# SegataLab/metamlst

Hardware: AMD Instinct MI355X
Metric: Mreads/s aligned+ST-typed, metamlstDB_2022; ST concordance vs CPU ref (higher is better)
Workload: dtype int32

## Files before the change

### metamlst_amd/csrc/mlst_engine.hip

```cpp
#include <hip/hip_runtime.h>
#include <algorithm>
#include <cmath>
#include <cstdarg>
#include <cstdio>
#include <cstdlib>
#include <cstring>
#include <cstddef>
#include <functional>
#include <atomic>
#include <memory>
#include <mutex>
#include <string>
#include <thread>
#include <vector>
#include <chrono>
#include <unistd.h>

#include "mlst.h"
#include "mlst_debug.h"
#include "bgzf_host.h"
#include "inflate_dev.h"
#include "inflate_wave.h"
#include "inflate_lane.h"
#include "inflate_canon.h"
// ... 91 lines not shown
    u64 sv_wgmax;
    u64 cnt[MLST_CNT_N];
    u64 rt_next;
    u64 rt_parked;
    u64 rt_ring_full;
    u64 pad_[13];
    u64 ext_q2[EXT_Q][16];
};
#define IS_SINGLE 1
#define IS_DONE   2
#define IS_ACC    4
struct KParams {
    int minscore, max_xm, min_read_len, minqual, match_bonus, n_penalty, open_p, ext_p, gbar, band_w, trig, quirk, clip;
};
#if defined(__HIP_DEVICE_COMPILE__)
#define GLOBAL_AS __attribute__((address_space(1)))
#else
#define GLOBAL_AS
#endif
template <typename T> struct GP {
    T* p;
#if defined(__HIP_DEVICE_COMPILE__)
    typedef __attribute__((address_space(1))) T G;
#else
    typedef T G;
#endif
    __host__ __device__ GP& operator=(T* q) { p = q; return *this; }
    template <typename I> __device__ G& operator[](I i) const { return ((G*)p)[i]; }
    __device__ G* operator->() const { return (G*)p; }
    __host__ __device__ operator T*() const { return p; }
    __device__ G* g() const { return (G*)p; }
};

struct EngineDev {
    GP<const u32> arena; GP<const u32> planes; GP<const u32> nmask; GP<const u16> allele_len; GP<const u32> allele_locus; GP<const LocusDev> loci;
    GP<const uint4> sieve; u32 sieve_mask;
    GP<const u32> bitmap;
    GP<const u32> gbitmap; u32 gbitmap_bits;
    GP<const u64> keys; GP<const u32> vals; GP<const u32> posts; u32 table_mask;
    GP<const int> floor_tab; GP<const u8> pen_tab;
    u32 n_alleles, n_loci;
    GP<const HapRec> hap_rec; GP<const u32> hap_blk; GP<const u32> hap_id;
    GP<u64> acc64;
    GP<long long> sum_score; GP<u32> n_hits; GP<u64> locus_len; GP<u64> locus_first;
    GP<Counters> ctr;
    GP<u32> ret_bases; GP<u8> ret_quals; GP<u16> ret_len; GP<u64> ret_ridx; GP<u32> ret_nrec;
    GP<u32> ret_cpos;
    GP<u32> ret_mate; GP<u32> ret_item0; GP<u8> ret_nitems;
    GP<ItemDev> items; GP<u8> item_state; GP<u32> res; GP<u64> dp_list;
    u64 cap_ret, cap_items, cap_res, cap_dp;
};

#define TIE1(a)             asm volatile("" : "+v"(a))
#define TIE4(a, b, c, d)    asm volatile("" : "+v"(a), "+v"(b), "+v"(c), "+v"(d))
#define TIE7(a, b, c, d, e, f, g) asm volatile("" : "+v"(a), "+v"(b), "+v"(c), "+v"(d), "+v"(e), "+v"(f), "+v"(g))
template <int N, typename T> __device__ inline void tie_all(T (&v)[N]) {
    #pragma unroll
    for (int i = 0; i + 4 <= N; i += 4) TIE4(v[i], v[i + 1], v[i + 2], v[i + 3]);
    #pragma unroll
    for (int i = N - (N % 4); i < N; i++) TIE1(v[i]);
}

__device__ inline u64 uniform_u64(u64 v) {
    return ((u64)(u32)__builtin_amdgcn_readfirstlane((u32)(v >> 32)) << 32) | (u64)(u32)__builtin_amdgcn_readfirstlane((u32)v);
}

__host__ __device__ inline u64 packed_index(u64 r, u32 wpr, u32 c) {
    return (r >> 6) * 64 * wpr + ((((u64)(c >> 1)) * 64 + (r & 63)) << 1) + (c & 1);
}
__host__ __device__ inline u64 packed_words(u64 n_reads, u32 wpr) { return ((n_reads + 63) & ~63ull) * wpr; }

template <u32 QB, typename LenFn>
__device__ inline void pack_group(const u8* __restrict__ bases, const u8* __restrict__ quals, const u64* __restrict__ seq_off,
                                  const u64* __restrict__ qual_off, LenFn len_of, u64 n_reads, u64 grp,
                                  u32* __restrict__ packed, u8* __restrict__ qrows, u16* __restrict__ lens, u32 wpr, u32 qstride,
                                  u32* s_words , u32* s_anyn ) {
    const int tid = threadIdx.x;
    if (tid < 2) s_anyn[tid] = 0;
// ... 1836 lines not shown
#define XT_ITEM xt_items++
#define XT_FLUSH do { if ((threadIdx.x & 63) == 0) { for (int k_ = 0; k_ < 6; k_++) atomicAdd(&g_ext_trace[k_], xt_[k_]); atomicAdd(&g_ext_trace[6], xt_items); atomicAdd(&g_ext_trace[7], 1ull); } } while (0)
#else
#define XT_DECL const u32 xskip_ = __builtin_amdgcn_readfirstlane(g_ext_skip)
#define XT(k)
#define XT_ITEM
#define XT_FLUSH
#endif
extern "C" int mlst_debug_ext_trace(uint64_t out[8], int reset) {
    if (hipMemcpyFromSymbol(out, HIP_SYMBOL(g_ext_trace), 64) != hipSuccess) return -1;
    if (reset) { u64 z[8] = {0, 0, 0, 0, 0, 0, 0, 0}; if (hipMemcpyToSymbol(HIP_SYMBOL(g_ext_trace), z, 64) != hipSuccess) return -1; }
    return 0;
}
#else
#define XC(k, v)
#define XSKIP(b) false
#define XT_DECL
#define XT(k)
#define XT_ITEM
#define XT_FLUSH
#endif
#define R_TRACK 0x10000000u

template <int NB>
__device__ __forceinline__ void extend_body(const EngineDev* __restrict__ Ep, const KParams& P, const u32 lds_recs, const u32 acc_cap, const u32* __restrict__ xrec, const u64 cap_xrec) {
    typedef XRec<NB> X;
    const EngineDev& E = *Ep;
    extern __shared__ int4 s_hap[];
    __shared__ u32 s_rl[RW / 2 + 2]; __shared__ u32 s_rh[RW / 2 + 2]; __shared__ u32 s_rn[RW / 2 + 2]; __shared__ u32 s_odd[RW / 2 + 2];
    __shared__ u8 s_pen[RQ]; __shared__ u8 s_pentab[128];
    __shared__ u32 s_cnt[16][3];
    __shared__ __attribute__((aligned(16))) u32 s_x[2][X::WORDS];
    __shared__ u64 s_ii[2];
    const int tid = threadIdx.x, nthr = blockDim.x, nwv = blockDim.x >> 6;
    for (int i = tid; i < 128; i += nthr) s_pentab[i] = E.pen_tab[i];
    u64 c_tot = 0, c_ign = 0;
    u64 N;
    { const u64 b0 = E.ctr->items_done, e0 = E.ctr->n_items < E.cap_items ? E.ctr->n_items : E.cap_items; N = e0 - b0; if (N > cap_xrec) N = cap_xrec; }
    const u64 QB = (N + EXT_Q - 1) / EXT_Q;
    u32 myq = blockIdx.x % EXT_Q, tried = 0;
    auto place = [&](u32 q, u64 ticket) -> u64 { const u64 pl = (u64)q * QB + ticket; return (ticket < QB && pl < N) ? pl : N; };
    auto resolve = [&](u64 ticket) -> u64 {
        u64 nx = place(myq, ticket);
        while (nx >= N && ++tried < EXT_Q) {
            myq = (myq + 1) % EXT_Q;
            const u64 seen = __hip_atomic_load((u64*)&E.ctr->ext_q[myq][0], __ATOMIC_RELAXED, __HIP_MEMORY_SCOPE_AGENT);
            nx = place(myq, seen) < N ? place(myq, atomicAdd(&E.ctr->ext_q[myq][0], 1ull)) : N;
        }
        if (nx < N) tried = 0;
        return nx;
    };
    if (tid == 0) {
        s_ii[0] = resolve(atomicAdd(&E.ctr->ext_q[myq][0], 1ull));
        s_ii[1] = tried < EXT_Q ? resolve(atomicAdd(&E.ctr->ext_q[myq][0], 1ull)) : N;
    }
    u16* const s_pend = reinterpret_cast<u16*>(s_hap + lds_recs + 1);
    const bool packed_acc = E.cap_items < (1ull << 24);
    __syncthreads();
    u64 pp = uniform_u64(s_ii[0]);
    if (pp < N) for (int j = tid; j < X::WORDS; j += nthr) s_x[0][j] = xrec[pp * X::WORDS + j];
    __syncthreads();
    int cur = 0;
    XT_DECL;
    while (pp < N) {
        XT_ITEM;
        const u64 pp_next = uniform_u64(s_ii[cur ^ 1]);
        u32 pf[(X::WORDS + 63) / 64];
        #pragma unroll
        for (int k = 0; k < (X::WORDS + 63) / 64; k++) { pf[k] = 0; if (pp_next < N && tid + 64 * k < X::WORDS && tid < 64) pf[k] = xrec[pp_next * X::WORDS + tid + 64 * k]; }
        u64 ticket = 0;
        if (tid == 0 && tried < EXT_Q) ticket = atomicAdd(&E.ctr->ext_q[myq][0], 1ull);
        asm volatile("" ::: "memory");
        const u32* x = s_x[cur];
        const uint4 h0 = *reinterpret_cast<const uint4*>(x), h1 = *reinterpret_cast<const uint4*>(x + 4), h2 = *reinterpret_cast<const uint4*>(x + 8), h3 = *reinterpret_cast<const uint4*>(x + 12);
        const u32 flags = __builtin_amdgcn_readfirstlane(h0.x);
        const u64 ii = (u64)(u32)__builtin_amdgcn_readfirstlane(x[31]);
        const int n = __builtin_amdgcn_readfirstlane(h0.y & 0xFFFFu), pen_def = __builtin_amdgcn_readfirstlane(h0.y >> 16);
        const int diag = __builtin_amdgcn_readfirstlane((int)h0.z);
        const u32 ret = __builtin_amdgcn_readfirstlane(h0.w);
        const u64 res_off = ((u64)(u32)__builtin_amdgcn_readfirstlane(h1.z) << 32) | (u32)__builtin_amdgcn_readfirstlane(h1.y);
        const u32 a_begin = __builtin_amdgcn_readfirstlane(h1.w), n_alleles = __builtin_amdgcn_readfirstlane(h2.x), n_pad = __builtin_amdgcn_readfirstlane(h2.y);
        const int floor_n = __builtin_amdgcn_readfirstlane((int)h3.y);
        const bool res_ok = flags & XF_RESOK, read_has_n = flags & XF_READN;
        const bool use_hap = res_ok && (flags & XF_HAPOK) && (u32)__builtin_amdgcn_readfirstlane(h3.w) <= lds_recs;
        u32 nrec = 0, ndp = 0, ntrack = 0;
        bool parked = false;
        auto park = [&]() {
            #pragma unroll
            for (int k = 0; k < (X::WORDS + 63) / 64; k++) if (tid < 64 && tid + 64 * k < X::WORDS) s_x[cur ^ 1][tid + 64 * k] = pf[k];
            if (tid == 0) s_ii[cur] = tried < EXT_Q ? resolve(ticket) : N;
            parked = true;
        };
        auto emit_pair = [&](const u32 a, const int score, const int xm, const int xo, bool need_dp, const bool valid) {
            u32 r = pack_result(score, xm, xo);
            need_dp = need_dp && valid;
            const bool is_rec = valid && !need_dp && score >= floor_n && score > 0;
            if (need_dp) r |= R_NEEDDP; else if (is_rec) r |= R_REC;
            nrec += (u32)__popcll(__ballot(is_rec));
            const u64 wm = __ballot(need_dp);
            if (wm) {
                ndp += (u32)__popcll(wm);
                int lane = tid & 63, leader = __ffsll((long long)wm) - 1; u64 base = 0;
                if (lane == leader) base = atomicAdd(&E.ctr->n_dp, (u64)__popcll(wm));
                base = __shfl(base, leader);
                if (need_dp) { u64 slot = base + __popcll(wm & ((1ull << lane) - 1));
                               if (slot < E.cap_dp) E.dp_list[slot] = (ii << 20) | (u64)a; else atomicOr(&E.ctr->err, 8ull); }
            }
            if (valid) E.res[res_off + a] = r;
        };
        auto stage_old = [&]() {
            ItemDev it; it.res_off = res_off; it.ret = ret; it.locus = __builtin_amdgcn_readfirstlane(h1.x); it.diag = diag; it.strand = (flags & XF_STRAND) ? 1 : 0; it.votes = 0;
            __syncthreads();
            stage_read_planes(E, P, it, n, s_rl, s_rh, s_rn, s_odd, s_pen, s_pentab, tid, nthr);
            __syncthreads();
        };
        auto pairs_loop = [&](const bool only_marked) {
            const LocusDev L = E.loci[__builtin_amdgcn_readfirstlane(h1.x)];
            u32 rl[NB], rh[NB], od[NB], rn[NB];
            #pragma unroll
            for (int w = 0; w < NB; w++) {
                rl[w] = __builtin_amdgcn_readfirstlane(s_rl[w]); rh[w] = __builtin_amdgcn_readfirstlane(s_rh[w]);
                od[w] = __builtin_amdgcn_readfirstlane(s_odd[w]);
                rn[w] = read_has_n ? __builtin_amdgcn_readfirstlane(s_rn[w]) : 0u;
            }
            for (u32 a = tid; a < n_alleles; a += nthr) {
                const bool valid = !only_marked || (E.res[res_off + a] & R_TRACK);
                int m = (int)E.allele_len[a_begin + a];
                int mm = 0, bs = 0, be = 0, best = P0;
                if (valid) best = L.has_n ? ungapped_planes<NB, false, true>(E, P, L, a, m, n, diag, rl, rh, od, rn, s_pen, pen_def, read_has_n, mm, bs, be)
                                         : ungapped_planes<NB, false, false>(E, P, L, a, m, n, diag, rl, rh, od, rn, s_pen, pen_def, read_has_n, mm, bs, be);
                const int score = best >> MLST_P_SHIFT, xm = 255 - (best & 0xFF), xo = 127 - ((best >> 8) & 0x7F);
                bool need_dp = P.trig < 0;
                if (valid && !need_dp && mm > P.trig && score >= floor_n) {
                    if (L.has_n) ungapped_planes<NB, true, true>(E, P, L, a, m, n, diag, rl, rh, od, rn, s_pen, pen_def, read_has_n, mm, bs, be);
                    else ungapped_planes<NB, true, false>(E, P, L, a, m, n, diag, rl, rh, od, rn, s_pen, pen_def, read_has_n, mm, bs, be);
                    need_dp = gap_trigger(P, mm, xm, score, floor_n, m, n, diag, bs, be);
                }
                emit_pair(a, score, xm, xo, need_dp, valid);
            }
        };
        XT(0);
        bool done_fast = false;
        if (use_hap) {
            const int q0 = diag >> 5;
            const u32 pblocks = __builtin_amdgcn_readfirstlane(h3.z);
            const u64 hid_off = ((u64)(u32)__builtin_amdgcn_readfirstlane(h3.x) << 32) | (u32)__builtin_amdgcn_readfirstlane(h2.w);
            constexpr int NR = (NB + 3) / 2;
            GP<const u32>::G* idrow[NR];
            #pragma unroll
            for (int j = 0; j < NR; j++) { int r = (q0 >> 1) + j; const int nrows = (int)((pblocks + 1) >> 1); r = r < 0 ? 0 : (r >= nrows ? nrows - 1 : r); idrow[j] = E.hap_id.g() + hid_off + (u64)(u32)r * n_pad; }
            const u32 odd16 = ((u32)q0 & 1u) * 16u;
            auto load_ids = [&](const u32 a, u32 (&w)[NR]) {
                const u32 ac = a < n_alleles ? a : n_alleles - 1;
                if (XSKIP(8u)) { for (int j = 0; j < NR; j++) w[j] = 0; return; }
                #pragma unroll
                for (int j = 0; j < NR; j++) w[j] = ld_row(idrow[j], ac * 4u);
            };
            u32 hb[NB + 2];
            #pragma unroll
            for (int t = 0; t <= NB + 1; t++) hb[t] = __builtin_amdgcn_readfirstlane(x[X::HB + t]);
            auto recs = E.hap_rec.g() + __builtin_amdgcn_readfirstlane(h2.z);
            u32 maxcnt = 0;
            #pragma unroll
            for (int t = 0; t <= NB; t++) { const u32 c = hb[t + 1] - hb[t]; maxcnt = c > maxcnt ? c : maxcnt; }
            const bool special_any = flags & XF_SPECIAL;
            if (special_any) {
                auto rq = E.ret_quals.g() + (u64)ret * RQ;
                for (int i = tid; i < n; i += nthr) { const u8 qb = rq[(flags & XF_STRAND) ? n - 1 - i : i]; s_pen[i] = (qb >> 7) ? (u8)P.n_penalty : s_pentab[qb & 0x7F]; }
            }
            u32 Wn[NR], Wn2[NR], Wn3[NR], Wn4[NR];
            load_ids((u32)tid, Wn); load_ids((u32)tid + nthr, Wn2); load_ids((u32)tid + 2 * nthr, Wn3); load_ids((u32)tid + 3 * nthr, Wn4);
            const u32 ident = hb[NB + 1] - hb[0];
            u32 sbase[NB + 1], wid[NB + 1];
            #pragma unroll
            for (int t = 0; t <= NB; t++) { const bool present = hb[t + 1] != hb[t]; sbase[t] = present ? hb[t] - hb[0] : ident; wid[t] = present ? 16u : 0u; }
            if (tid == 0) s_hap[ident] = make_int4(0, NEGP, NEGP, NEGP);
            if (special_any) lds_barrier();
            XT(1);
            for (u32 hb0 = 0; hb0 < maxcnt && !XSKIP(1u); hb0 += nthr) {
                const u32 hh = hb0 + tid;
                uint4 rc[NB + 1];
                #pragma unroll
                for (int t = 0; t <= NB; t++) {
                    rc[t] = make_uint4(0, 0, 0, 0);
                    if (hh < hb[t + 1] - hb[t]) rc[t] = *reinterpret_cast<GP<const uint4>::G*>(recs + hb[t] + hh);
                }
                #pragma unroll
                for (int t = 0; t <= NB; t++) { TIE4(rc[t].x, rc[t].y, rc[t].z, rc[t].w); }
                #pragma unroll
                for (int t = 0; t <= NB; t++) {
                    if (hh < hb[t + 1] - hb[t]) {
                        const uint4 sp = *reinterpret_cast<const uint4*>(x + X::PL + 4 * t); HapRec hr; hr.lo = rc[t].x; hr.hi = rc[t].y; hr.nm = rc[t].z; hr.len = rc[t].w;
                        s_hap[(hb[t] - hb[0]) + hh] = hap_summary(P, hr, sp.x, sp.y, sp.z, sp.w, x[X::VR + t], s_pen, 32 * t - (int)((u32)diag & 31u), pen_def, special_any);
                    }
                }
            }
            park();
            lds_barrier();
            XT(2);
            auto compose = [&](const u32 (&w)[NR], int& best, int& mm) {
                u32 wp[NB / 2 + 1];
                #pragma unroll
                for (int k = 0; k <= NB / 2; k++) wp[k] = __builtin_amdgcn_alignbit(k + 1 < NR ? w[k + 1 < NR ? k + 1 : 0] : 0u, w[k], odd16);
                int4 S[NB + 1];
                #pragma unroll
                for (int t = 0; t <= NB; t++) S[t] = s_hap[sbase[t] + __builtin_amdgcn_ubfe(wp[t >> 1], 16u * (t & 1), wid[t])];
                int v = P0, ts = 0; best = P0;
                #pragma unroll
                for (int t = 0; t <= NB; t++) {
                    const int c1 = v + S[t].z; best = c1 > best ? c1 : best; best = S[t].w > best ? S[t].w : best;
                    const int c2 = v + S[t].x; v = c2 > S[t].y ? c2 : S[t].y; ts += S[t].x;
                }
                best = v > best ? v : best;
                mm = (-ts) & 0xFFFF;
            };
            auto span_needs_dp = [&](const u32 (&w)[NR], const int mm, const int xm, const int score) -> bool {
                const int MA = P.match_bonus << MLST_P_SHIFT, PD = (pen_def << MLST_P_SHIFT) + 1;
                int cur = P0, best = P0, cs = 0, last = 0, blen = 0, overlap = 0, i1 = 0; bool first = true;
                #pragma unroll
                for (int t = 0; t <= NB; t++) {
                    if (hb[t + 1] == hb[t]) continue;
                    const u32 k = (u32)t + (odd16 >> 4);
                    const u32 id = (w[k >> 1] >> (16u * (k & 1u))) & 0xFFFFu;
                    const uint4 rc = *reinterpret_cast<GP<const uint4>::G*>(recs + hb[t] + id);
                    const uint4 sp = *reinterpret_cast<const uint4*>(x + X::PL + 4 * t);
                    const u32 lm = rc.w >= 32u ? 0xFFFFFFFFu : ((1u << rc.w) - 1u), valid = x[X::VR + t] & lm;
                    if (!valid) continue;
                    u32 M = ((rc.x ^ sp.x) | (rc.y ^ sp.y) | sp.z | rc.z) & valid;
                    const int lo_c = __ffs((int)valid) - 1, nv = __popc(valid);
                    if (first) { cs = last = 32 * t + lo_c; first = false; }
                    overlap += nv; i1 = 32 * t + lo_c + nv;
                    const u32 special = sp.w | rc.z;
                    while (M) {
                        const int bit = __ffs((int)M) - 1; M &= M - 1;
                        const int i = 32 * t + bit;
                        cur += (i - last) * MA;
                        if (cur > best) { best = cur; blen = i - cs; }
                        int dec = PD;
                        if ((special >> bit) & 1u) dec = ((((rc.z >> bit) & 1u) ? P.n_penalty : (int)s_pen[32 * t - (int)((u32)diag & 31u) + bit]) << MLST_P_SHIFT) + 1;
                        cur -= dec;
                        if (cur <= P0) { cur = P0; cs = i + 1; }
                        last = i + 1;
                    }
                }
                cur += (i1 - last) * MA;
                if (cur > best) blen = i1 - cs;
                const int clipped = overlap - blen;
                return mm > P.trig && score >= floor_n && clipped >= P.clip && 2 * (mm - xm) >= clipped;
            };
            const bool single = (flags & XF_SINGLE) != 0;
            bool slow = P.trig < 0 || n_alleles > acc_cap;
            if (!slow) {
                u16* const s_acc = s_pend;
                const bool n_ok = n >= P.min_read_len;
                u32 nacc = 0;
                for (u32 a = tid; a < n_alleles && !XSKIP(2u); a += nthr) {
                    u32 W[NR];
                    #pragma unroll
                    for (int j = 0; j < NR; j++) { W[j] = Wn[j]; Wn[j] = Wn2[j]; Wn2[j] = Wn3[j]; Wn3[j] = Wn4[j]; }
                    load_ids(a + 4 * nthr, Wn4);
                    asm volatile("" ::: "memory");
                    int best, mm; compose(W, best, mm);
                    const int score = best >> MLST_P_SHIFT, xm = 255 - (best & 0xFF);
                    const bool cand = score >= floor_n && score > 0;
                    bool track = cand && mm > P.trig;
                    if (track) track = span_needs_dp(W, mm, xm, score);
                    const bool rec = cand && !track, ok = rec && n_ok && score >= P.minscore && xm <= P.max_xm;
                    nrec += (u32)__popcll(__ballot(rec)); nacc += (u32)__popcll(__ballot(ok)); ntrack += (u32)__popcll(__ballot(track));
                    s_acc[a] = ok ? (u16)score : (u16)0;
                }
                u32 tot_rec = __builtin_amdgcn_readfirstlane(nrec), tot_acc = __builtin_amdgcn_readfirstlane(nacc), tot_track = __builtin_amdgcn_readfirstlane(ntrack);
                if (nwv > 1) {
                    if ((tid & 63) == 0) { s_cnt[tid >> 6][0] = tot_rec; s_cnt[tid >> 6][1] = tot_acc; s_cnt[tid >> 6][2] = tot_track; }
                    __syncthreads();
                    tot_rec = tot_acc = tot_track = 0;
                    for (int w = 0; w < nwv; w++) { tot_rec += s_cnt[w][0]; tot_acc += s_cnt[w][1]; tot_track += s_cnt[w][2]; }
                    __syncthreads();
                }
                if (tot_track == 0 && !(P.quirk && tot_rec == 1)) {
                    if (tot_acc) for (u32 a = tid; a < n_alleles; a += nthr) {
                        const u32 sc = s_acc[a];
                        if (sc && !XSKIP(4u)) {
                            if (packed_acc) atomicAdd(&E.acc64[a_begin + a], (1ull << 40) | (u64)sc);
                            else { atomicAdd((u64*)&E.sum_score[a_begin + a], (u64)sc); atomicAdd(&E.n_hits[a_begin + a], 1u); }
                        }
                    }
                    if (tid == 0) {
                        if (tot_rec) atomicAdd(&E.ret_nrec[ret], tot_rec);
                        c_tot += tot_rec; c_ign += tot_rec - tot_acc;
                        E.item_state[ii] = (u8)((single ? IS_SINGLE : 0) | IS_DONE | (tot_acc ? IS_ACC : 0));
                    }
                    done_fast = true;
                } else { slow = true; nrec = 0; ntrack = 0; }
            }
            if (slow) {
                load_ids((u32)tid, Wn);
                for (u32 a = tid; a < n_alleles; a += nthr) {
                    u32 W[NR];
                    #pragma unroll
                    for (int j = 0; j < NR; j++) W[j] = Wn[j];
                    load_ids(a + nthr, Wn);
                    asm volatile("" ::: "memory");
                    int best, mm; compose(W, best, mm);
                    const int score = best >> MLST_P_SHIFT, xm = 255 - (best & 0xFF), xo = 127 - ((best >> 8) & 0x7F);
                    const bool track = P.trig >= 0 && mm > P.trig && score >= floor_n;
                    const u64 tm = __ballot(track);
                    if (tm) { ntrack += (u32)__popcll(tm); if (track) E.res[res_off + a] = R_TRACK; }
                    emit_pair(a, score, xm, xo, P.trig < 0, !track);
                }
                ntrack = __builtin_amdgcn_readfirstlane(ntrack);
                if (nwv > 1) {
                    if ((tid & 63) == 0) s_cnt[tid >> 6][2] = ntrack;
                    __syncthreads();
                    ntrack = 0; for (int w = 0; w < nwv; w++) ntrack += s_cnt[w][2];
                }
                if (ntrack) { stage_old(); pairs_loop(true); }
            }
        }
// ... 21 lines not shown
            __syncthreads();
            if (tid == 0) {
                u32 A = 0, I = 0;
                for (int w = 0; w < nwv; w++) { A += s_cnt[w][0]; I += s_cnt[w][1]; }
                c_tot += tot_rec; c_ign += I;
                const u8 state = (u8)((flags & XF_SINGLE) ? IS_SINGLE : 0);
                E.item_state[ii] = (u8)(state | IS_DONE | (A ? IS_ACC : 0));
            }
        }
        }
        XT(4);
        if (!parked) park();
        lds_barrier();
        pp = pp_next; cur ^= 1;
        XT(5);
    }
    XT_FLUSH;
    if (tid == 0) {
        if (c_tot) atomicAdd(&E.ctr->cnt[MLST_CNT_TOTAL_RECORDS], c_tot);
        if (c_ign) atomicAdd(&E.ctr->cnt[MLST_CNT_IGNORED], c_ign);
    }
}

__global__ __launch_bounds__(1024) void k_extend_160(const EngineDev* __restrict__ Ep, KParams P, u32 lds_recs, u32 acc_cap, const u32* __restrict__ xrec, u64 cap_xrec) { extend_body<5>(Ep, P, lds_recs, acc_cap, xrec, cap_xrec); }
__global__ __launch_bounds__(512) void k_extend_320(const EngineDev* __restrict__ Ep, KParams P, u32 lds_recs, u32 acc_cap, const u32* __restrict__ xrec, u64 cap_xrec) { extend_body<RW / 2>(Ep, P, lds_recs, acc_cap, xrec, cap_xrec); }

template <int CTRL, int ROW_MASK = 0xF> __device__ inline int dpp_i32(int old, int src) {
    return __builtin_amdgcn_update_dpp(old, src, CTRL, ROW_MASK, 0xF, false);
}
__device__ inline int seg32_prefix_max(int v) {
    int t;
    t = dpp_i32<DPP_ROW_SHR(1)>(NEGP, v); v = t > v ? t : v;
    t = dpp_i32<DPP_ROW_SHR(2)>(NEGP, v); v = t > v ? t : v;
    t = dpp_i32<DPP_ROW_SHR(4)>(NEGP, v); v = t > v ? t : v;
    t = dpp_i32<DPP_ROW_SHR(8)>(NEGP, v); v = t > v ? t : v;
    t = dpp_i32<DPP_ROW_BCAST15, 0xA>(NEGP, v); v = t > v ? t : v;
    return v;
}

template <bool TRACE>
__device__ inline int banded(const EngineDev& E, const KParams& P, const ItemDev& it, const LocusDev& L, u32 a_local,
                             int n, const u8* s_pentab, u8* TB, int& bi, int& bb) {
    const int W = P.band_w, BW = 2 * W + 1, G = P.gbar, d = it.diag;
    const int m = (int)E.allele_len[L.a_begin + a_local];
    const int OPEN = P.open_p, EXT = P.ext_p, MA = P.match_bonus << MLST_P_SHIFT;
    auto rb = E.ret_bases.g() + (u64)it.ret * RW;
    auto rq = E.ret_quals.g() + (u64)it.ret * RQ;
    int Hp[2 * MAX_W + 2], Fp[2 * MAX_W + 2];
// ... 709 lines not shown
#include "read_overlap.h"
#include "read_filter.h"
#include "read_stats.h"
#include "aln_text.h"
#include "reads_text.h"

struct EvPair { hipEvent_t a, b; int which; };

struct mlst_handle {
    int device = 0;
    hipStream_t stream = nullptr;
    mlst_params prm;
    KParams kp;
    std::string err;
    std::vector<LocusDev> loci;
    std::vector<u64> aoff;
    u32 n_alleles = 0, n_loci = 0;
    std::vector<u32> allele_locus;
    u32* d_arena = nullptr; u32* d_planes = nullptr; u32* d_nmask = nullptr; u16* d_allele_len = nullptr; u32* d_allele_locus = nullptr;
    LocusDev* d_loci = nullptr; uint4* d_sieve = nullptr; u32* d_bitmap = nullptr; u32* d_gbitmap = nullptr; u64* d_keys = nullptr; u32* d_vals = nullptr; u32* d_posts = nullptr;
    int* d_floor = nullptr; u8* d_pen = nullptr; u8* d_ascii = nullptr; u64* d_aoff = nullptr;
    HapRec* d_hap_rec = nullptr; u32* d_hap_blk = nullptr; u32* d_hap_id = nullptr; u64 bytes_hap = 0, n_hap_rec = 0; u32 hap_win_max[2] = {0, 0}, hap_loci = 0;
    u32 ext_lds_recs[2] = {0, 0};
    u32 ext_acc_cap = 0;
    u8* h_qc = nullptr; u8* d_qc = nullptr; u64 cap_hostq = 0, cap_qc = 0;
    u64* d_acc64 = nullptr;
    u32* d_xrec[2] = {nullptr, nullptr}; u64 cap_xrec[2] = {0, 0};
    u64 bytes_arena = 0, bytes_sieve = 0, bytes_table = 0; double bitmap_fill = 0.0;
    EngineDev E; EngineDev* d_E = nullptr;
    bool have_ref = false, have_state = false;
    u32* d_cand = nullptr; u64 cap_cand = 0;
    int sieve_kind = 0; u32 sieve_chain = 0; u64 n_keys = 0;
    u32* d_rfilter = nullptr; u32* d_rt_arena = nullptr; u64 cap_rt_arena = 0; u32* d_rt_counts = nullptr; u32* d_rt_emitted = nullptr; u64 cap_rt_emitted = 0;
    u32 rt_prod = 0, rt_cap = 0, rt_tiles_max = 0, rt_nw = 16, rt_pf = 2, rt_exam = RT_EXAM_DEFAULT, rt_wo = 1; u64 rt_slice = 0;
    u64* d_rt_parked = nullptr; u64 cap_rt_parked = 0;
    u64* d_rt_trace = nullptr; bool rt_trace_on = false; const void* rt_last_packed = nullptr;
    std::vector<void*> dbg_pads;
    u32* d_bin_flags = nullptr; u64 cap_bin_flags = 0;
    u8* d_in_bases = nullptr; u8* d_in_quals = nullptr; u64* d_in_off = nullptr; u64 cap_in_bytes = 0, cap_in_reads = 0;
    u32* d_packed = nullptr; u8* d_qrows = nullptr; u16* d_lens = nullptr; u64 cap_packed_words = 0, cap_qrow_bytes = 0, cap_lens = 0;
    u64 reads_seen = 0;
    u32 max_wpr = 0;
    int ext_threads = 64, ext_blocks = 5120;
    int extp_threads = 256, extp_blocks = 1792; u32 pair_loci = 0;
    int sieve_g_blocks = 256 * 5;
    u8* d_fq_text = nullptr;
// ... 720 lines not shown
        std::vector<LocusDev> lc = loci;
        u32 mx_hap = 0, mx_pair = 0, n_hap = 0, n_pair = 0; h->hap_win_max[0] = h->hap_win_max[1] = 0;
        for (auto& L : lc) {
            const bool take = L.hap_ok && L.n_alleles <= hap_max && (u64)L.hap_win[1] * 16 <= (u64)budget_kb * 1024;
            L.hap_ok = take ? 1u : 0u;
            if (take) { n_hap++; mx_hap = std::max(mx_hap, L.n_alleles); for (int k = 0; k < 2; k++) h->hap_win_max[k] = std::max(h->hap_win_max[k], L.hap_win[k]); }
            else { n_pair++; mx_pair = std::max(mx_pair, L.n_alleles); }
        }
        h->loci = lc; h->hap_loci = n_hap; h->pair_loci = n_pair;
        HIPCHK(h, hipMemcpy(h->d_loci, lc.data(), (u64)n_loci * sizeof(LocusDev), hipMemcpyHostToDevice));
        int thr = mx_hap <= 512 ? 64 : 256;
        const char* e1 = getenv("MLST_EXT_THREADS"); if (e1 && atoi(e1) >= 64 && atoi(e1) <= 1024 && atoi(e1) % 64 == 0) thr = atoi(e1);
        int blocks = 1280 * 256 / thr;
        const char* e2 = getenv("MLST_EXT_BLOCKS"); if (e2 && atoi(e2) > 0) blocks = atoi(e2);
        h->ext_threads = thr; h->ext_blocks = blocks;
        int thr2 = mx_pair <= 512 ? 64 : 256;
        const char* e5 = getenv("MLST_EXTP_THREADS"); if (e5 && atoi(e5) >= 64 && atoi(e5) <= 1024 && atoi(e5) % 64 == 0) thr2 = atoi(e5);
        int blocks2 = 1792 * 256 / thr2;
        const char* e6 = getenv("MLST_EXTP_BLOCKS"); if (e6 && atoi(e6) > 0) blocks2 = atoi(e6);
        h->extp_threads = thr2; h->extp_blocks = blocks2;
        h->ext_acc_cap = std::min<u32>((mx_hap + 63u) & ~63u, 16384u);
        for (int k = 0; k < 2; k++) {
            h->ext_lds_recs[k] = h->hap_win_max[k];
            if (ext_lds_bytes(h, k) > 48u * 1024u)
                HIPCHK(h, hipFuncSetAttribute(k ? (const void*)k_extend_320 : (const void*)k_extend_160, hipFuncAttributeMaxDynamicSharedMemorySize, (int)ext_lds_bytes(h, k)));
        }
        const char* e3 = getenv("MLST_SIEVE_BLOCKS"); if (e3 && atoi(e3) > 0) h->sieve_g_blocks = atoi(e3);
        const char* e7 = getenv("MLST_RT_SLICE"); h->rt_slice = (e7 && atoll(e7) > 0) ? (u64)atoll(e7) : 0;
    }
    h->have_ref = h->have_state = true;
    int rc = reset_sample_state(h); if (rc) return rc;
    HIPCHK(h, hipStreamSynchronize(h->stream));
    return MLST_OK;
}

extern "C" int mlst_set_read_index_base(mlst_handle* h, uint64_t base) {
    if (!h || !h->have_state) return fail(h, MLST_E_INVALID, "no reference loaded");
    h->reads_seen = base;
    return MLST_OK;
}

extern "C" int mlst_reset_sample(mlst_handle* h) {
    if (!h || !h->have_state) return fail(h, MLST_E_INVALID, "no reference loaded");
    hipSetDevice(h->device);
    drain_events(h);
    if (h->bz_pend.on || h->bzp.on) { if (h->infl_stream) hipStreamSynchronize(h->infl_stream); h->bz_pend.on = false; h->bzp.on = false; }
    return reset_sample_state(h);
}

// ... 69 lines not shown
    if (!h || !h->have_state) return fail(h, MLST_E_INVALID, "no reference loaded");
    hipSetDevice(h->device);
    if (wpr == 0 || wpr > RW || (wpr & 1)) return fail(h, MLST_E_INVALID, "words_per_read must be even and in 2..%d", RW);
    if (qstride < 4 || qstride > RQ || (qstride & 3)) return fail(h, MLST_E_INVALID, "qual_stride must be a multiple of 4 in 4..%d", RQ);
    if (phase != 1 && (!d_qrows || ((uintptr_t)d_qrows & 3) != 0)) return fail(h, MLST_E_INVALID, "quality rows must be 4-byte aligned");
    if (n_reads >= (1ull << 32)) return fail(h, MLST_E_LIMIT, "a batch holds at most 2^32-1 reads");
    if (((uintptr_t)d_packed & 15) != 0) return fail(h, MLST_E_INVALID, "packed rows must be 16-byte aligned");
    if (n_reads == 0) return MLST_OK;
    paired = paired ? 1 : 0;
    if (paired && ((n_reads | h->reads_seen) & 1ull)) return fail(h, MLST_E_INVALID, "paired submissions hold whole pairs (reads 2k, 2k+1) and start at an even read index");
    if (h->cap_cand < n_reads) { hipStreamSynchronize(h->stream); hipFree(h->d_cand); h->d_cand = nullptr; HIPCHK(h, dmalloc(&h->d_cand, n_reads)); h->cap_cand = n_reads; }
    EngineDev& E = h->E;
    if (wpr > h->max_wpr) h->max_wpr = wpr;
    u64 rt_slice = 0;
    if (h->sieve_kind == MLST_SIEVE_ROUTED && h->rt_slice) { rt_slice = (h->rt_slice + 1023) & ~1023ull; if (rt_slice >= n_reads) rt_slice = 0; }
    if (h->sieve_kind == MLST_SIEVE_ROUTED) { int rc = ensure_route_buffers(h, rt_slice ? rt_slice : n_reads, wpr, n_reads); if (rc) return rc; }
    {
        const int k = wpr <= 10 ? 0 : 1; const u64 words = k ? (u64)XRec<RW / 2>::WORDS : (u64)XRec<5>::WORDS;
        if (h->hap_loci && !h->d_xrec[k]) { hipStreamSynchronize(h->stream); HIPCHK(h, dmalloc(&h->d_xrec[k], h->E.cap_items * words)); h->cap_xrec[k] = h->E.cap_items; }
    }
    const int gs = phase ? 0 : graph_enter(h, h->g_submit, {(u64)(uintptr_t)d_packed, (u64)(uintptr_t)d_qrows, (u64)(uintptr_t)d_lens, (u64)n_reads, (u64)wpr,
                                               (u64)qstride, (u64)h->reads_seen, (u64)(uintptr_t)h->d_cand,
                                               (u64)(uintptr_t)h->d_bin_flags, (u64)(uintptr_t)h->d_rt_arena, (u64)(uintptr_t)h->d_rt_counts,
                                               (u64)(uintptr_t)h->d_rt_emitted, (u64)h->rt_cap, (u64)h->rt_prod, (u64)h->rt_nw, (u64)paired, (u64)(uintptr_t)h->d_rt_trace, (u64)(uintptr_t)h->d_rt_parked, (u64)h->cap_rt_parked, (u64)h->rt_pf, rt_slice, (u64)h->rt_exam, (u64)h->rt_wo});
    if (gs == 1) { h->reads_seen += n_reads; return MLST_OK; }
    if (phase != 2) { Prof pf(h, 0);
      if (h->sieve_kind == MLST_SIEVE_LDS) {
        dim3 grid(grid_for((n_reads + 1023) / 1024, 1, 256)), block(1024);
#define SIEVE_CASE(W) case W: hipLaunchKernelGGL((k_sieve_q<W, true>), grid, block, 0, h->stream, d_packed, d_lens, (u64)n_reads, E.sieve, E.sieve_mask, E.bitmap, 0u, h->d_cand, E.ctr, paired); break;
        switch (wpr) { SIEVE_CASE(2) SIEVE_CASE(4) SIEVE_CASE(6) SIEVE_CASE(8) SIEVE_CASE(10) SIEVE_CASE(12) SIEVE_CASE(14)
                       SIEVE_CASE(16) SIEVE_CASE(18) SIEVE_CASE(20) default: return fail(h, MLST_E_INVALID, "words_per_read %u unsupported", wpr); }
#undef SIEVE_CASE
      } else if (h->sieve_kind == MLST_SIEVE_ROUTED) {
        const u64 n_flag_words = (n_reads + 31) >> 5;
        for (u64 sl_first = 0; sl_first < n_reads; sl_first += (rt_slice ? rt_slice : n_reads)) {
        const u64 sl_n = rt_slice ? std::min<u64>(rt_slice, n_reads - sl_first) : n_reads;
        const u32* sl_packed = d_packed + (sl_first >> 6) * 64 * wpr; const u16* sl_lens = d_lens + sl_first;
        if (sl_first) hipLaunchKernelGGL(k_rt_reset, dim3(1), dim3(1), 0, h->stream, E.ctr);
        RouteDev R; R.arena = h->d_rt_arena; R.counts = h->d_rt_counts; R.emitted = h->d_rt_emitted; R.filter = h->d_rfilter; R.flags = h->d_bin_flags + (sl_first >> 5); R.trace = h->d_rt_trace; R.parked = h->d_rt_parked; R.parked_cap = h->cap_rt_parked;
        h->rt_last_packed = d_packed;
        R.cap = h->rt_cap; R.n_prod = h->rt_prod; R.tiles_max = h->rt_tiles_max; R.nw = h->rt_nw;
        { const char* e = getenv("MLST_RT_DEBUG"); R.dbg = e ? (u32)atoi(e) : 0u; if (R.dbg & 2u) R.parked_cap = 0; }
        { Prof pa(h, 9);
#define ROUTE_LAUNCH(W, N, WO) hipLaunchKernelGGL((k_route<W, N, WO>), dim3(h->rt_prod), dim3(N * 64), 0, h->stream, sl_packed, sl_lens, (u64)sl_n, R, E.ctr)
#define SIEVE_CASE(W) case W: if (h->rt_nw == 8) { if (h->rt_wo) ROUTE_LAUNCH(W, 8, true); else ROUTE_LAUNCH(W, 8, false); } \
                              else { if (h->rt_wo) ROUTE_LAUNCH(W, 16, true); else ROUTE_LAUNCH(W, 16, false); } break;
        switch (wpr) { SIEVE_CASE(2) SIEVE_CASE(4) SIEVE_CASE(6) SIEVE_CASE(8) SIEVE_CASE(10) SIEVE_CASE(12) SIEVE_CASE(14)
// ... 16 lines not shown
                       SIEVE_CASE(16) SIEVE_CASE(18) SIEVE_CASE(20) default: return fail(h, MLST_E_INVALID, "words_per_read %u unsupported", wpr); }
#undef SIEVE_CASE
        }
        }
        hipLaunchKernelGGL(k_flag_compact, dim3(grid_for((n_flag_words + FLAG_U - 1) / FLAG_U, 1024, 512)), dim3(1024), 0, h->stream, h->d_bin_flags, (u64)n_reads, h->d_cand, E.ctr, paired);
      } else {
        dim3 grid(grid_for((n_reads + 255) / 256, 1, h->sieve_g_blocks)), block(256);
#define SIEVE_CASE(W) case W: hipLaunchKernelGGL((k_sieve_q<W, false>), grid, block, 0, h->stream, d_packed, d_lens, (u64)n_reads, E.sieve, E.sieve_mask, E.gbitmap.p, E.gbitmap_bits, h->d_cand, E.ctr, paired); break;
        switch (wpr) { SIEVE_CASE(2) SIEVE_CASE(4) SIEVE_CASE(6) SIEVE_CASE(8) SIEVE_CASE(10) SIEVE_CASE(12) SIEVE_CASE(14)
                       SIEVE_CASE(16) SIEVE_CASE(18) SIEVE_CASE(20) default: return fail(h, MLST_E_INVALID, "words_per_read %u unsupported", wpr); }
#undef SIEVE_CASE
      }
    }
    if (phase == 1) { HIPCHK(h, hipGetLastError()); return MLST_OK; }
    { Prof pf(h, 1);
      hipLaunchKernelGGL(k_seed, dim3(1024), dim3(256), 0, h->stream, h->d_E, d_packed, d_qrows, d_lens, wpr, qstride, h->reads_seen, h->d_cand, paired, phase == 2 ? 1 : 0);
      hipLaunchKernelGGL(k_retain, dim3(2048), dim3(256), 0, h->stream, h->d_E, d_packed, d_qrows, wpr, qstride, h->reads_seen, phase == 2 ? 1 : 0); }
    if (h->hap_loci) {
      { Prof pf(h, 12);
        if (wpr <= 10) hipLaunchKernelGGL(k_ext_prep<5>, dim3(2048), dim3(256), 0, h->stream, h->d_E, h->kp, h->d_xrec[0], h->cap_xrec[0]);
        else hipLaunchKernelGGL(k_ext_prep<RW / 2>, dim3(2048), dim3(256), 0, h->stream, h->d_E, h->kp, h->d_xrec[1], h->cap_xrec[1]); }
      { Prof pf(h, 2);
        const int thr = h->ext_threads, blocks = h->ext_blocks;
        if (wpr <= 10) hipLaunchKernelGGL(k_extend_160, dim3(blocks), dim3(thr), ext_lds_bytes(h, 0), h->stream, h->d_E, h->kp, h->ext_lds_recs[0], h->ext_acc_cap, h->d_xrec[0], h->cap_xrec[0]);
        else hipLaunchKernelGGL(k_extend_320, dim3(blocks), dim3(std::min(thr, 512)), ext_lds_bytes(h, 1), h->stream, h->d_E, h->kp, h->ext_lds_recs[1], h->ext_acc_cap, h->d_xrec[1], h->cap_xrec[1]); }
    }
    if (h->pair_loci) { Prof pf(h, 2);
      const int thr = h->extp_threads, blocks = h->extp_blocks;
      if (wpr <= 10) hipLaunchKernelGGL(k_extend_pairs_160, dim3(blocks), dim3(thr), 0, h->stream, h->d_E, h->kp);
      else hipLaunchKernelGGL(k_extend_pairs_320, dim3(blocks), dim3(thr), 0, h->stream, h->d_E, h->kp); }
    { Prof pf(h, 3); hipLaunchKernelGGL(k_banded, dim3(1024), dim3(256), 0, h->stream, h->d_E, h->kp); }
    { Prof pf(h, 4); hipLaunchKernelGGL(k_accumulate, dim3(1024), dim3(256), 0, h->stream, h->d_E, h->kp);
      hipLaunchKernelGGL(k_locus, dim3(128), dim3(1024), 0, h->stream, h->d_E, paired); }
    hipLaunchKernelGGL(k_advance, dim3(1), dim3(1), 0, h->stream, E.ctr, n_reads);
    if (gs == 2) { int rc = graph_leave(h, h->g_submit); if (rc) return rc; }
    HIPCHK(h, hipGetLastError());
    h->reads_seen += n_reads;
    return MLST_OK;
}

static int ensure_pack_buffers(mlst_handle* h, u64 n_reads, u32 wpr, u32 qstride) {
    h->last_pack.n_reads = 0; h->last_pack.wpr = h->last_pack.qstride = 0;
    if (h->cap_packed_words < packed_words(n_reads, wpr) + 4 || h->cap_qrow_bytes < n_reads * qstride || h->cap_lens < n_reads + 2) {
        hipStreamSynchronize(h->stream);
        hipFree(h->d_packed); hipFree(h->d_qrows); hipFree(h->d_lens); h->d_packed = nullptr; h->d_qrows = nullptr; h->d_lens = nullptr;
        HIPCHK(h, dmalloc(&h->d_packed, packed_words(n_reads, wpr) + 4)); HIPCHK(h, dmalloc(&h->d_qrows, n_reads * qstride)); HIPCHK(h, dmalloc(&h->d_lens, n_reads + 2));
        h->cap_packed_words = packed_words(n_reads, wpr) + 4; h->cap_qrow_bytes = n_reads * qstride; h->cap_lens = n_reads + 2;
    }
// ... 2820 lines not shown
```

Baseline: 21360.

## Read extend item records via scalar constant-address loads instead of LDS staging

Adds an SREC variant of the extend kernel that reads each item's record directly from global memory through address-space-4 (constant) pointers, so fields come in as scalar loads. It drops the cooperative LDS copy, the per-item prefetch into registers, and the __syncthreads that went with them. Fields are reloaded lazily at their points of use, with the pointer pinned to SGPRs to lower register pressure. This becomes the default, and an environment variable restores the LDS path. In exchange, scalar loads may miss cache and add latency on the critical path, since the next record is no longer prefetched.

After: 21050. 0.985x the previous value.

```diff
diff --git a/metamlst_amd/csrc/mlst_engine.hip b/metamlst_amd/csrc/mlst_engine.hip
--- a/metamlst_amd/csrc/mlst_engine.hip
+++ b/metamlst_amd/csrc/mlst_engine.hip
@@ -137,14 +137,17 @@
     T* p;
 #if defined(__HIP_DEVICE_COMPILE__)
     typedef __attribute__((address_space(1))) T G;
+    typedef __attribute__((address_space(4))) T K;
 #else
     typedef T G;
+    typedef T K;
 #endif
     __host__ __device__ GP& operator=(T* q) { p = q; return *this; }
     template <typename I> __device__ G& operator[](I i) const { return ((G*)p)[i]; }
     __device__ G* operator->() const { return (G*)p; }
     __host__ __device__ operator T*() const { return p; }
     __device__ G* g() const { return (G*)p; }
+    __device__ static K* k(T* q) { return (K*)q; }
 };
 
 struct EngineDev {
@@ -169,6 +172,11 @@
 #define TIE1(a)             asm volatile("" : "+v"(a))
 #define TIE4(a, b, c, d)    asm volatile("" : "+v"(a), "+v"(b), "+v"(c), "+v"(d))
 #define TIE7(a, b, c, d, e, f, g) asm volatile("" : "+v"(a), "+v"(b), "+v"(c), "+v"(d), "+v"(e), "+v"(f), "+v"(g))
+#if defined(__HIP_DEVICE_COMPILE__)
+#define TIE_S(p)            asm volatile("" : "+s"(p))
+#else
+#define TIE_S(p)
+#endif
 template <int N, typename T> __device__ inline void tie_all(T (&v)[N]) {
     #pragma unroll
     for (int i = 0; i + 4 <= N; i += 4) TIE4(v[i], v[i + 1], v[i + 2], v[i + 3]);
@@ -2051,15 +2059,16 @@
 #endif
 #define R_TRACK 0x10000000u
 
-template <int NB>
+template <int NB, bool SREC>
 __device__ __forceinline__ void extend_body(const EngineDev* __restrict__ Ep, const KParams& P, const u32 lds_recs, const u32 acc_cap, const u32* __restrict__ xrec, const u64 cap_xrec) {
     typedef XRec<NB> X;
+    typedef typename GP<const u32>::K* XK;
     const EngineDev& E = *Ep;
     extern __shared__ int4 s_hap[];
     __shared__ u32 s_rl[RW / 2 + 2]; __shared__ u32 s_rh[RW / 2 + 2]; __shared__ u32 s_rn[RW / 2 + 2]; __shared__ u32 s_odd[RW / 2 + 2];
     __shared__ u8 s_pen[RQ]; __shared__ u8 s_pentab[128];
     __shared__ u32 s_cnt[16][3];
-    __shared__ __attribute__((aligned(16))) u32 s_x[2][X::WORDS];
+    __shared__ __attribute__((aligned(16))) u32 s_x[2][SREC ? 4 : X::WORDS];
     __shared__ u64 s_ii[2];
     const int tid = threadIdx.x, nthr = blockDim.x, nwv = blockDim.x >> 6;
     for (int i = tid; i < 128; i += nthr) s_pentab[i] = E.pen_tab[i];
@@ -2087,36 +2096,53 @@
     const bool packed_acc = E.cap_items < (1ull << 24);
     __syncthreads();
     u64 pp = uniform_u64(s_ii[0]);
-    if (pp < N) for (int j = tid; j < X::WORDS; j += nthr) s_x[0][j] = xrec[pp * X::WORDS + j];
-    __syncthreads();
+    if constexpr (!SREC) {
+        if (pp < N) for (int j = tid; j < X::WORDS; j += nthr) s_x[0][j] = xrec[pp * X::WORDS + j];
+        __syncthreads();
+    }
     int cur = 0;
     XT_DECL;
     while (pp < N) {
         XT_ITEM;
         const u64 pp_next = uniform_u64(s_ii[cur ^ 1]);
         u32 pf[(X::WORDS + 63) / 64];
-        #pragma unroll
-        for (int k = 0; k < (X::WORDS + 63) / 64; k++) { pf[k] = 0; if (pp_next < N && tid + 64 * k < X::WORDS && tid < 64) pf[k] = xrec[pp_next * X::WORDS + tid + 64 * k]; }
+        if constexpr (!SREC) {
+            #pragma unroll
+            for (int k = 0; k < (X::WORDS + 63) / 64; k++) { pf[k] = 0; if (pp_next < N && tid + 64 * k < X::WORDS && tid < 64) pf[k] = xrec[pp_next * X::WORDS + tid + 64 * k]; }
+        }
         u64 ticket = 0;
         if (tid == 0 && tried < EXT_Q) ticket = atomicAdd(&E.ctr->ext_q[myq][0], 1ull);
         asm volatile("" ::: "memory");
-        const u32* x = s_x[cur];
-        const uint4 h0 = *reinterpret_cast<const uint4*>(x), h1 = *reinterpret_cast<const uint4*>(x + 4), h2 = *reinterpret_cast<const uint4*>(x + 8), h3 = *reinterpret_cast<const uint4*>(x + 12);
-        const u32 flags = __builtin_amdgcn_readfirstlane(h0.x);
-        const u64 ii = (u64)(u32)__builtin_amdgcn_readfirstlane(x[31]);
-        const int n = __builtin_amdgcn_readfirstlane(h0.y & 0xFFFFu), pen_def = __builtin_amdgcn_readfirstlane(h0.y >> 16);
-        const int diag = __builtin_amdgcn_readfirstlane((int)h0.z);
-        const u32 ret = __builtin_amdgcn_readfirstlane(h0.w);
-        const u64 res_off = ((u64)(u32)__builtin_amdgcn_readfirstlane(h1.z) << 32) | (u32)__builtin_amdgcn_readfirstlane(h1.y);
-        const u32 a_begin = __builtin_amdgcn_readfirstlane(h1.w), n_alleles = __builtin_amdgcn_readfirstlane(h2.x), n_pad = __builtin_amdgcn_readfirstlane(h2.y);
-        const int floor_n = __builtin_amdgcn_readfirstlane((int)h3.y);
+        const u32* x = s_x[SREC ? 0 : cur];
+        uint4 h0 = make_uint4(0, 0, 0, 0), h1 = h0, h2 = h0, h3 = h0;
+        if constexpr (!SREC) { h0 = *reinterpret_cast<const uint4*>(x); h1 = *reinterpret_cast<const uint4*>(x + 4); h2 = *reinterpret_cast<const uint4*>(x + 8); h3 = *reinterpret_cast<const uint4*>(x + 12); }
+        const XK xk = GP<const u32>::k(xrec + pp * X::WORDS);
+        auto at = [&]() -> XK { XK p = xk; if constexpr (SREC) TIE_S(p); return p; };
+        auto XW = [&](const XK p, const int j) -> u32 {
+            if constexpr (SREC) return p[j];
+            else {
+                if (j >= 16) return (u32)__builtin_amdgcn_readfirstlane(x[j]);
+                const uint4 h = j < 4 ? h0 : (j < 8 ? h1 : (j < 12 ? h2 : h3));
+                return (u32)__builtin_amdgcn_readfirstlane((j & 3) == 0 ? h.x : ((j & 3) == 1 ? h.y : ((j & 3) == 2 ? h.z : h.w)));
+            }
+        };
+        const XK p_top = at();
+        const u32 flags = XW(p_top, 0), w_n = XW(p_top, 1), n_alleles = XW(p_top, 8);
+        const int n = (int)(w_n & 0xFFFFu), pen_def = (int)(w_n >> 16);
+        const int diag = (int)XW(p_top, 2), floor_n = (int)XW(p_top, 13);
         const bool res_ok = flags & XF_RESOK, read_has_n = flags & XF_READN;
-        const bool use_hap = res_ok && (flags & XF_HAPOK) && (u32)__builtin_amdgcn_readfirstlane(h3.w) <= lds_recs;
+        const bool use_hap = res_ok && (flags & XF_HAPOK) && XW(p_top, 15) <= lds_recs;
+        u64 ii = 0, res_off = 0; u32 ret = 0, a_begin = 0;
+        auto load_dest = [&](const XK p) { ret = XW(p, 3); a_begin = XW(p, 7); ii = (u64)XW(p, 31); };
+        auto load_res = [&](const XK p) { res_off = ((u64)XW(p, 6) << 32) | (u64)XW(p, 5); };
+        if constexpr (!SREC) { load_dest(p_top); load_res(p_top); }
         u32 nrec = 0, ndp = 0, ntrack = 0;
         bool parked = false;
         auto park = [&]() {
-            #pragma unroll
-            for (int k = 0; k < (X::WORDS + 63) / 64; k++) if (tid < 64 && tid + 64 * k < X::WORDS) s_x[cur ^ 1][tid + 64 * k] = pf[k];
+            if constexpr (!SREC) {
+                #pragma unroll
+                for (int k = 0; k < (X::WORDS + 63) / 64; k++) if (tid < 64 && tid + 64 * k < X::WORDS) s_x[cur ^ 1][tid + 64 * k] = pf[k];
+            }
             if (tid == 0) s_ii[cur] = tried < EXT_Q ? resolve(ticket) : N;
             parked = true;
         };
@@ -2138,13 +2164,13 @@
             if (valid) E.res[res_off + a] = r;
         };
         auto stage_old = [&]() {
-            ItemDev it; it.res_off = res_off; it.ret = ret; it.locus = __builtin_amdgcn_readfirstlane(h1.x); it.diag = diag; it.strand = (flags & XF_STRAND) ? 1 : 0; it.votes = 0;
+            ItemDev it; it.res_off = res_off; it.ret = ret; it.locus = XW(at(), 4); it.diag = diag; it.strand = (flags & XF_STRAND) ? 1 : 0; it.votes = 0;
             __syncthreads();
             stage_read_planes(E, P, it, n, s_rl, s_rh, s_rn, s_odd, s_pen, s_pentab, tid, nthr);
             __syncthreads();
         };
         auto pairs_loop = [&](const bool only_marked) {
-            const LocusDev L = E.loci[__builtin_amdgcn_readfirstlane(h1.x)];
+            const LocusDev L = E.loci[XW(at(), 4)];
             u32 rl[NB], rh[NB], od[NB], rn[NB];
             #pragma unroll
             for (int w = 0; w < NB; w++) {
@@ -2172,8 +2198,9 @@
         bool done_fast = false;
         if (use_hap) {
             const int q0 = diag >> 5;
-            const u32 pblocks = __builtin_amdgcn_readfirstlane(h3.z);
-            const u64 hid_off = ((u64)(u32)__builtin_amdgcn_readfirstlane(h3.x) << 32) | (u32)__builtin_amdgcn_readfirstlane(h2.w);
+            const XK p_hap = at();
+            const u32 pblocks = XW(p_hap, 14), n_pad = XW(p_hap, 9);
+            const u64 hid_off = ((u64)XW(p_hap, 12) << 32) | (u64)XW(p_hap, 11);
             constexpr int NR = (NB + 3) / 2;
             GP<const u32>::G* idrow[NR];
             #pragma unroll
@@ -2187,14 +2214,14 @@
             };
             u32 hb[NB + 2];
             #pragma unroll
-            for (int t = 0; t <= NB + 1; t++) hb[t] = __builtin_amdgcn_readfirstlane(x[X::HB + t]);
-            auto recs = E.hap_rec.g() + __builtin_amdgcn_readfirstlane(h2.z);
+            for (int t = 0; t <= NB + 1; t++) hb[t] = XW(p_hap, X::HB + t);
+            auto recs = E.hap_rec.g() + XW(p_hap, 10);
             u32 maxcnt = 0;
             #pragma unroll
             for (int t = 0; t <= NB; t++) { const u32 c = hb[t + 1] - hb[t]; maxcnt = c > maxcnt ? c : maxcnt; }
             const bool special_any = flags & XF_SPECIAL;
             if (special_any) {
-                auto rq = E.ret_quals.g() + (u64)ret * RQ;
+                auto rq = E.ret_quals.g() + (u64)XW(p_hap, 3) * RQ;
                 for (int i = tid; i < n; i += nthr) { const u8 qb = rq[(flags & XF_STRAND) ? n - 1 - i : i]; s_pen[i] = (qb >> 7) ? (u8)P.n_penalty : s_pentab[qb & 0x7F]; }
             }
             u32 Wn[NR], Wn2[NR], Wn3[NR], Wn4[NR];
@@ -2216,11 +2243,15 @@
                 }
                 #pragma unroll
                 for (int t = 0; t <= NB; t++) { TIE4(rc[t].x, rc[t].y, rc[t].z, rc[t].w); }
+                const XK p_pl = at();
                 #pragma unroll
                 for (int t = 0; t <= NB; t++) {
                     if (hh < hb[t + 1] - hb[t]) {
-                        const uint4 sp = *reinterpret_cast<const uint4*>(x + X::PL + 4 * t); HapRec hr; hr.lo = rc[t].x; hr.hi = rc[t].y; hr.nm = rc[t].z; hr.len = rc[t].w;
-                        s_hap[(hb[t] - hb[0]) + hh] = hap_summary(P, hr, sp.x, sp.y, sp.z, sp.w, x[X::VR + t], s_pen, 32 * t - (int)((u32)diag & 31u), pen_def, special_any);
+                        uint4 sp; u32 vr;
+                        if constexpr (SREC) { sp = make_uint4(p_pl[X::PL + 4 * t], p_pl[X::PL + 4 * t + 1], p_pl[X::PL + 4 * t + 2], p_pl[X::PL + 4 * t + 3]); vr = p_pl[X::VR + t]; }
+                        else { sp = *reinterpret_cast<const uint4*>(x + X::PL + 4 * t); vr = x[X::VR + t]; }
+                        HapRec hr; hr.lo = rc[t].x; hr.hi = rc[t].y; hr.nm = rc[t].z; hr.len = rc[t].w;
+                        s_hap[(hb[t] - hb[0]) + hh] = hap_summary(P, hr, sp.x, sp.y, sp.z, sp.w, vr, s_pen, 32 * t - (int)((u32)diag & 31u), pen_def, special_any);
                     }
                 }
             }
@@ -2244,16 +2275,23 @@
                 mm = (-ts) & 0xFFFF;
             };
             auto span_needs_dp = [&](const u32 (&w)[NR], const int mm, const int xm, const int score) -> bool {
-                const int MA = P.match_bonus << MLST_P_SHIFT, PD = (pen_def << MLST_P_SHIFT) + 1;
+                const XK p_pl = at();
+                const int diag_w = SREC ? (int)XW(p_pl, 2) : diag, pen_def_w = SREC ? (int)(XW(p_pl, 1) >> 16) : pen_def;
+                const u32 odd16_w = SREC ? ((u32)(diag_w >> 5) & 1u) * 16u : odd16;
+                auto recs_w = SREC ? E.hap_rec.g() + XW(p_pl, 10) : recs;
+                const int MA = P.match_bonus << MLST_P_SHIFT, PD = (pen_def_w << MLST_P_SHIFT) + 1;
                 int cur = P0, best = P0, cs = 0, last = 0, blen = 0, overlap = 0, i1 = 0; bool first = true;
                 #pragma unroll
                 for (int t = 0; t <= NB; t++) {
-                    if (hb[t + 1] == hb[t]) continue;
-                    const u32 k = (u32)t + (odd16 >> 4);
+                    const u32 hb_t = SREC ? XW(p_pl, X::HB + t) : hb[t], hb_t1 = SREC ? XW(p_pl, X::HB + t + 1) : hb[t + 1];
+                    if (hb_t1 == hb_t) continue;
+                    const u32 k = (u32)t + (odd16_w >> 4);
                     const u32 id = (w[k >> 1] >> (16u * (k & 1u))) & 0xFFFFu;
-                    const uint4 rc = *reinterpret_cast<GP<const uint4>::G*>(recs + hb[t] + id);
-                    const uint4 sp = *reinterpret_cast<const uint4*>(x + X::PL + 4 * t);
-                    const u32 lm = rc.w >= 32u ? 0xFFFFFFFFu : ((1u << rc.w) - 1u), valid = x[X::VR + t] & lm;
+                    const uint4 rc = *reinterpret_cast<GP<const uint4>::G*>(recs_w + hb_t + id);
+                    uint4 sp; u32 vr;
+                    if constexpr (SREC) { sp = make_uint4(p_pl[X::PL + 4 * t], p_pl[X::PL + 4 * t + 1], p_pl[X::PL + 4 * t + 2], p_pl[X::PL + 4 * t + 3]); vr = p_pl[X::VR + t]; }
+                    else { sp = *reinterpret_cast<const uint4*>(x + X::PL + 4 * t); vr = x[X::VR + t]; }
+                    const u32 lm = rc.w >= 32u ? 0xFFFFFFFFu : ((1u << rc.w) - 1u), valid = vr & lm;
                     if (!valid) continue;
                     u32 M = ((rc.x ^ sp.x) | (rc.y ^ sp.y) | sp.z | rc.z) & valid;
                     const int lo_c = __ffs((int)valid) - 1, nv = __popc(valid);
@@ -2266,7 +2304,7 @@
                         cur += (i - last) * MA;
                         if (cur > best) { best = cur; blen = i - cs; }
                         int dec = PD;
-                        if ((special >> bit) & 1u) dec = ((((rc.z >> bit) & 1u) ? P.n_penalty : (int)s_pen[32 * t - (int)((u32)diag & 31u) + bit]) << MLST_P_SHIFT) + 1;
+                        if ((special >> bit) & 1u) dec = ((((rc.z >> bit) & 1u) ? P.n_penalty : (int)s_pen[32 * t - (int)((u32)diag_w & 31u) + bit]) << MLST_P_SHIFT) + 1;
                         cur -= dec;
                         if (cur <= P0) { cur = P0; cs = i + 1; }
                         last = i + 1;
@@ -2307,6 +2345,7 @@
                     __syncthreads();
                 }
                 if (tot_track == 0 && !(P.quirk && tot_rec == 1)) {
+                    if constexpr (SREC) load_dest(at());
                     if (tot_acc) for (u32 a = tid; a < n_alleles; a += nthr) {
                         const u32 sc = s_acc[a];
                         if (sc && !XSKIP(4u)) {
@@ -2323,6 +2362,7 @@
                 } else { slow = true; nrec = 0; ntrack = 0; }
             }
             if (slow) {
+                if constexpr (SREC) { const XK p_slow = at(); load_dest(p_slow); load_res(p_slow); }
                 load_ids((u32)tid, Wn);
                 for (u32 a = tid; a < n_alleles; a += nthr) {
                     u32 W[NR];
@@ -2390,8 +2430,10 @@
     }
 }
 
-__global__ __launch_bounds__(1024) void k_extend_160(const EngineDev* __restrict__ Ep, KParams P, u32 lds_recs, u32 acc_cap, const u32* __restrict__ xrec, u64 cap_xrec) { extend_body<5>(Ep, P, lds_recs, acc_cap, xrec, cap_xrec); }
-__global__ __launch_bounds__(512) void k_extend_320(const EngineDev* __restrict__ Ep, KParams P, u32 lds_recs, u32 acc_cap, const u32* __restrict__ xrec, u64 cap_xrec) { extend_body<RW / 2>(Ep, P, lds_recs, acc_cap, xrec, cap_xrec); }
+template <bool SREC>
+__global__ __launch_bounds__(1024) void k_extend_160(const EngineDev* __restrict__ Ep, KParams P, u32 lds_recs, u32 acc_cap, const u32* __restrict__ xrec, u64 cap_xrec) { extend_body<5, SREC>(Ep, P, lds_recs, acc_cap, xrec, cap_xrec); }
+template <bool SREC>
+__global__ __launch_bounds__(512) void k_extend_320(const EngineDev* __restrict__ Ep, KParams P, u32 lds_recs, u32 acc_cap, const u32* __restrict__ xrec, u64 cap_xrec) { extend_body<RW / 2, SREC>(Ep, P, lds_recs, acc_cap, xrec, cap_xrec); }
 
 template <int CTRL, int ROW_MASK = 0xF> __device__ inline int dpp_i32(int old, int src) {
     return __builtin_amdgcn_update_dpp(old, src, CTRL, ROW_MASK, 0xF, false);
@@ -3147,6 +3189,7 @@
     int* d_floor = nullptr; u8* d_pen = nullptr; u8* d_ascii = nullptr; u64* d_aoff = nullptr;
     HapRec* d_hap_rec = nullptr; u32* d_hap_blk = nullptr; u32* d_hap_id = nullptr; u64 bytes_hap = 0, n_hap_rec = 0; u32 hap_win_max[2] = {0, 0}, hap_loci = 0;
     u32 ext_lds_recs[2] = {0, 0};
+    u32 ext_srec = 1;
     u32 ext_acc_cap = 0;
     u8* h_qc = nullptr; u8* d_qc = nullptr; u64 cap_hostq = 0, cap_qc = 0;
     u64* d_acc64 = nullptr;
@@ -3913,9 +3956,12 @@
         h->ext_acc_cap = std::min<u32>((mx_hap + 63u) & ~63u, 16384u);
         for (int k = 0; k < 2; k++) {
             h->ext_lds_recs[k] = h->hap_win_max[k];
-            if (ext_lds_bytes(h, k) > 48u * 1024u)
-                HIPCHK(h, hipFuncSetAttribute(k ? (const void*)k_extend_320 : (const void*)k_extend_160, hipFuncAttributeMaxDynamicSharedMemorySize, (int)ext_lds_bytes(h, k)));
-        }
+            if (ext_lds_bytes(h, k) > 48u * 1024u) {
+                HIPCHK(h, hipFuncSetAttribute(k ? (const void*)k_extend_320<true> : (const void*)k_extend_160<true>, hipFuncAttributeMaxDynamicSharedMemorySize, (int)ext_lds_bytes(h, k)));
+                HIPCHK(h, hipFuncSetAttribute(k ? (const void*)k_extend_320<false> : (const void*)k_extend_160<false>, hipFuncAttributeMaxDynamicSharedMemorySize, (int)ext_lds_bytes(h, k)));
+            }
+        }
+        { const char* e = getenv("MLST_EXT_RECORD"); h->ext_srec = (e && !strcmp(e, "lds")) ? 0u : 1u; }
         const char* e3 = getenv("MLST_SIEVE_BLOCKS"); if (e3 && atoi(e3) > 0) h->sieve_g_blocks = atoi(e3);
         const char* e7 = getenv("MLST_RT_SLICE"); h->rt_slice = (e7 && atoll(e7) > 0) ? (u64)atoll(e7) : 0;
     }
@@ -4031,7 +4077,7 @@
     const int gs = phase ? 0 : graph_enter(h, h->g_submit, {(u64)(uintptr_t)d_packed, (u64)(uintptr_t)d_qrows, (u64)(uintptr_t)d_lens, (u64)n_reads, (u64)wpr,
                                                (u64)qstride, (u64)h->reads_seen, (u64)(uintptr_t)h->d_cand,
                                                (u64)(uintptr_t)h->d_bin_flags, (u64)(uintptr_t)h->d_rt_arena, (u64)(uintptr_t)h->d_rt_counts,
-                                               (u64)(uintptr_t)h->d_rt_emitted, (u64)h->rt_cap, (u64)h->rt_prod, (u64)h->rt_nw, (u64)paired, (u64)(uintptr_t)h->d_rt_trace, (u64)(uintptr_t)h->d_rt_parked, (u64)h->cap_rt_parked, (u64)h->rt_pf, rt_slice, (u64)h->rt_exam, (u64)h->rt_wo});
+                                               (u64)(uintptr_t)h->d_rt_emitted, (u64)h->rt_cap, (u64)h->rt_prod, (u64)h->rt_nw, (u64)paired, (u64)(uintptr_t)h->d_rt_trace, (u64)(uintptr_t)h->d_rt_parked, (u64)h->cap_rt_parked, (u64)h->rt_pf, rt_slice, (u64)h->rt_exam, (u64)h->rt_wo, (u64)h->ext_srec});
     if (gs == 1) { h->reads_seen += n_reads; return MLST_OK; }
     if (phase != 2) { Prof pf(h, 0);
       if (h->sieve_kind == MLST_SIEVE_LDS) {
@@ -4094,8 +4140,11 @@
         else hipLaunchKernelGGL(k_ext_prep<RW / 2>, dim3(2048), dim3(256), 0, h->stream, h->d_E, h->kp, h->d_xrec[1], h->cap_xrec[1]); }
       { Prof pf(h, 2);
         const int thr = h->ext_threads, blocks = h->ext_blocks;
-        if (wpr <= 10) hipLaunchKernelGGL(k_extend_160, dim3(blocks), dim3(thr), ext_lds_bytes(h, 0), h->stream, h->d_E, h->kp, h->ext_lds_recs[0], h->ext_acc_cap, h->d_xrec[0], h->cap_xrec[0]);
-        else hipLaunchKernelGGL(k_extend_320, dim3(blocks), dim3(std::min(thr, 512)), ext_lds_bytes(h, 1), h->stream, h->d_E, h->kp, h->ext_lds_recs[1], h->ext_acc_cap, h->d_xrec[1], h->cap_xrec[1]); }
+#define EXTEND_LAUNCH(K, SREC, k, T) hipLaunchKernelGGL(K<SREC>, dim3(blocks), dim3(T), ext_lds_bytes(h, k), h->stream, h->d_E, h->kp, h->ext_lds_recs[k], h->ext_acc_cap, h->d_xrec[k], h->cap_xrec[k])
+        if (wpr <= 10) { if (h->ext_srec) EXTEND_LAUNCH(k_extend_160, true, 0, thr); else EXTEND_LAUNCH(k_extend_160, false, 0, thr); }
+        else { if (h->ext_srec) EXTEND_LAUNCH(k_extend_320, true, 1, std::min(thr, 512)); else EXTEND_LAUNCH(k_extend_320, false, 1, std::min(thr, 512)); }
+#undef EXTEND_LAUNCH
+      }
     }
     if (h->pair_loci) { Prof pf(h, 2);
       const int thr = h->extp_threads, blocks = h->extp_blocks;
```
